# sunshanlu/ORB_SLAM2_ROS2

Hardware: AMD Instinct MI355X
Metric: stereo frames/sec (extract+match) KITTI-00 1241x376; HBM GB/s vs roofline (higher is better)
Workload: dtype u8; 1 GPU; Single 1241x376 KITTI-shaped stereo pair, 8-level pyramid, 2000 FAST+rBRIEF keypoints per image, searchByStereo; batched (512 pairs per step, 512 of them distinct synthetic frames).  `value` is DEVICE-RESIDENT; the checks, rooflines, host_io, sequence job, content sweep, CPU baseline and extra legs run with --full; io=device-resident, n_features=2000, levels=8

## Files before the change

### orb_slam2_ros2_amd/csrc/k_brief.hip

```cpp
#include <hip/hip_runtime.h>
#include <cstdio>
#include <cstring>

#include "orb_math.h"
#include "orbfe_internal.h"
#ifdef BRIEF_STAMPS
namespace orbfe { extern __device__ unsigned long long g_rt_t[4][8]; }
#define RT_STAMP(k) { __syncthreads(); if (tid == 0 && blockIdx.y == 0) orbfe::g_rt_t[k][0] = __builtin_amdgcn_s_memrealtime(); }
#define RTP_STAMP(k) { __syncthreads(); if (tid == 0 && blockIdx.y == 0) orbfe::g_rt_t[k][r] = __builtin_amdgcn_s_memrealtime(); }
#endif
#include "rowtable_body.h"
#include "wave_ops.h"

namespace orbfe {

typedef unsigned long long UmaxPacked;

template <int CTRL, int ROW_MASK>
__device__ __forceinline__ int dpp_i32(int v) {
  return __builtin_amdgcn_update_dpp(0, v, CTRL, ROW_MASK, 0xf, false);
}
__device__ __forceinline__ int wave_sum_i(int v) {
  v += dpp_i32<0x111, 0xf>(v);
  v += dpp_i32<0x112, 0xf>(v);
// ... 247 lines not shown
  orbfe_keypoint kp;
  kp.x = (float)x * L.sf;
  kp.y = (float)y * L.sf;
  kp.size = 7.0f;
  kp.angle = (float)(theta / 3.14159265358979323846 * 180);
  kp.response = (float)((e.y >> 8) & 0xFFu);
  kp.octave = level;
  kp.class_id = -1;
  kps[o] = kp;
#ifndef EXP_NO_KPS_HOST
  if (kps_host) kps_host[o] = kp;
#endif
  kx[o] = kpx_of(kp, L.sf);
  const float r = (float)(2.0 * (double)L.sf);
  const unsigned row = (unsigned)__float2int_rn(kp.y);
  KpAux a;
  a.row_max = (int16_t)min(rows0, __float2int_rn((float)row + r + 1.0f));
  a.row_min = (int16_t)max(0, __float2int_rn((float)row - r));
  aux[o] = a;
  if (theta_out) theta_out[o] = theta;
}

#define BRIEF_R 18
#define BRIEF_ROWS (2 * BRIEF_R + 1)
#define BRIEF_PITCH 48
#define BRIEF_WIN_BYTES 2048

#ifndef BRIEF_WAVES
#define BRIEF_WAVES 4
#endif
#ifndef BRIEF_KPW
#define BRIEF_KPW 2
#endif
#ifdef BRIEF_STAMPS
__device__ unsigned long long g_rt_t[4][8];
__device__ unsigned long long g_bs_rec[8192][6];
#define BS_DECL const unsigned bs_w = ((blockIdx.y * 520u + blockIdx.x) * BRIEF_WAVES + (threadIdx.x >> 6)) & 8191u; const unsigned long long bs_t0 = __builtin_amdgcn_s_memrealtime(); unsigned long long bs_t1 = 0, bs_ta = 0, bs_tb = 0;
#define BS_MID if (!bs_t1) bs_t1 = __builtin_amdgcn_s_memrealtime();
#define BS_END(kind) if ((threadIdx.x & 63) == 0) { asm volatile("s_waitcnt vmcnt(0) lgkmcnt(0)" ::: "memory"); g_bs_rec[bs_w][0] = bs_t0, g_bs_rec[bs_w][1] = bs_t1, g_bs_rec[bs_w][2] = __builtin_amdgcn_s_memrealtime(), g_bs_rec[bs_w][3] = kind, g_bs_rec[bs_w][4] = bs_ta, g_bs_rec[bs_w][5] = bs_tb; }
#else
#define BS_DECL
#define BS_MID
#define BS_END(kind)
#endif
struct BriefRowTable {
  const KpAux* aux;
  const int32_t* n_kp;
  uint32_t* rowoff;
  uint16_t* rowlist;
  int32_t* n_match;
  int rows, list_cap, slot0, n_brief_blocks;
  int stage_cap;
  int32_t* flags;
};
__global__ __launch_bounds__(64 * BRIEF_WAVES) __attribute__((amdgpu_waves_per_eu(8, 8))) void k_brief(const uint8_t* __restrict__ blur, size_t img_pitch,
                                              const uint4* __restrict__ kpl, int n_features, const int8_t* __restrict__ pattern,
                                              const double2* __restrict__ sincos, uint8_t* __restrict__ desc, uint8_t* __restrict__ desc_host,
                                              BriefRowTable rt) {
#pragma clang fp contract(off)
  struct __attribute__((aligned(16))) Lds {
    double rc[BRIEF_WAVES][40];
    uint8_t win[BRIEF_WAVES][2][BRIEF_WIN_BYTES];
    double rs[BRIEF_WAVES][40];
  };
  static_assert(BRIEF_ROWS * BRIEF_PITCH <= BRIEF_WIN_BYTES && BRIEF_WIN_BYTES == 2 * 64 * 16 && BRIEF_PITCH % 16 == 0, "a window is two 16-byte LDS-DMA instructions");
  static_assert((sizeof(double) * 40 * BRIEF_WAVES) % 16 == 0, "the LDS-DMA destination is 16-byte aligned");
  static_assert(sizeof(double) * 40 * BRIEF_WAVES + 2 * BRIEF_WIN_BYTES * BRIEF_WAVES > 255 * 8 &&
                    (sizeof(double) * 40 * BRIEF_WAVES + 2 * BRIEF_WIN_BYTES * BRIEF_WAVES) % 512 != 0,
                "rc[w] and rs[w] must not be reachable by one ds_read2(st64)_b64");
  __shared__ Lds lds;
  BS_DECL
  if (rt.rowoff && (int)blockIdx.x >= rt.n_brief_blocks) {
    static_assert(sizeof(Lds) >= 9000, "the table's row counters borrow the descriptor kernel's LDS (launch_orient_brief checks the row count against 9000 bytes)");
    uint32_t* cnt = (uint32_t*)&lds;
    const int slot = rt.slot0 + (int)blockIdx.y;
    const int r = (int)blockIdx.x - rt.n_brief_blocks;
    if (rt.flags) {
      if (r == 0 && threadIdx.x == 0) rt.n_match[slot >> 1] = 0;
      const int rpw = (rt.rows + 7) >> 3;
      extern __shared__ __attribute__((aligned(16))) uint2 brief_bands[];
      rowtable_build_part(rt.aux + (size_t)blockIdx.y * n_features, min(rt.n_kp[blockIdx.y], n_features), rt.rows, rt.list_cap,
                          rt.rowoff + (size_t)slot * (rt.rows + 1), rt.rowlist + (size_t)slot * rt.list_cap, cnt, cnt + rpw + 12, (int)threadIdx.x, r,
                          rt.flags + (size_t)blockIdx.y * 8, rt.stage_cap > 0 ? brief_bands : nullptr, rt.stage_cap / 4);
      BS_END(2)
      return;
    }
    if (r != 0) return;
    if (threadIdx.x == 0) rt.n_match[slot >> 1] = 0;
    extern __shared__ __attribute__((aligned(16))) uint16_t brief_stage[];
    rowtable_build(rt.aux + (size_t)blockIdx.y * n_features, min(rt.n_kp[blockIdx.y], n_features), rt.rows, rt.list_cap,
                   rt.rowoff + (size_t)slot * (rt.rows + 1), rt.rowlist + (size_t)slot * rt.list_cap, cnt, cnt + rt.rows, (int)threadIdx.x,
                   rt.stage_cap > 0 ? brief_stage : nullptr, rt.stage_cap);
    BS_END(2)
    return;
  }
  const int lane = threadIdx.x & 63;
  const int wave = __builtin_amdgcn_readfirstlane((int)(threadIdx.x >> 6));
  double* rc = lds.rc[wave];
  double* rs = lds.rs[wave];
  const int per_xcd = rt.n_brief_blocks >> 3;
  const int kb = ((int)blockIdx.x & 7) * per_xcd + ((int)blockIdx.x >> 3);
  const int k0 = (kb * BRIEF_WAVES + wave) * BRIEF_KPW;
  const int img = blockIdx.y;
  if (k0 >= n_features) return;
  const uint4* list = kpl + (size_t)img * n_features;
  const double2* sc = sincos + (size_t)img * n_features;
  const uint8_t* W = blur + (size_t)img * img_pitch;
  const int k_last = min(k0 + BRIEF_KPW, n_features) - 1;
  uint32_t tp0 = *(const uint32_t*)(pattern + (0 * 64 + lane) * 4), tp1 = *(const uint32_t*)(pattern + (1 * 64 + lane) * 4);
  uint32_t tp2 = *(const uint32_t*)(pattern + (2 * 64 + lane) * 4), tp3 = *(const uint32_t*)(pattern + (3 * 64 + lane) * 4);
#ifdef BRIEF_STAMPS
  asm volatile("s_waitcnt vmcnt(0)" :: "v"(tp0), "v"(tp1), "v"(tp2), "v"(tp3) : "memory");
  bs_t1 = __builtin_amdgcn_s_memrealtime();
#endif
  const int u1 = min(lane + 64, BRIEF_ROWS * (BRIEF_PITCH / 16) - 1);
  const uint32_t row_a = (uint32_t)lane / 3u, row_b = (uint32_t)u1 / 3u;
  const uint32_t col_a = 16u * ((uint32_t)lane - 3u * row_a), col_b = 16u * ((uint32_t)u1 - 3u * row_b);
  typedef __attribute__((address_space(3))) uint8_t* lds_dst_t;
  typedef const __attribute__((address_space(1))) uint8_t* glb_src_t;
  auto request = [&](const uint4 e, int b) __attribute__((always_inline)) {
    const bool used = (e.x & 0xFFFFu) != 0xFFFFu;
    const int x = used ? (int)(e.x & 0xFFFFu) : BRIEF_R, y = used ? (int)(e.x >> 16) : BRIEF_R;
    const uint32_t plane = used ? e.z : 0u;
    const uint32_t stride = used ? e.w : 0u;
    const uint32_t xa = (uint32_t)(x - BRIEF_R) & ~3u;
    const uint32_t s0 = plane + (uint32_t)(y - BRIEF_R) * stride + xa;
    uint8_t* dst = lds.win[wave][b];
    __builtin_amdgcn_global_load_lds((glb_src_t)(W + (s0 + col_a + __umul24(row_a, stride))), (lds_dst_t)dst, 16, 0, 0);
    __builtin_amdgcn_global_load_lds((glb_src_t)(W + (s0 + col_b + __umul24(row_b, stride))), (lds_dst_t)(dst + 1024), 16, 0, 0);
  };
  uint4 e_cur = list[k0];
  uint4 e_nxt = list[min(k0 + 1, k_last)];
  double2 sc_cur = sc[k0];
#ifdef BRIEF_STAMPS
  asm volatile("s_waitcnt lgkmcnt(0)" ::: "memory");
  bs_ta = __builtin_amdgcn_s_memrealtime();
#endif
  asm volatile("" : "+v"(tp0), "+v"(tp1), "+v"(tp2), "+v"(tp3));
  request(e_cur, 0);
#ifdef BRIEF_STAMPS
  asm volatile("s_waitcnt vmcnt(0)" ::: "memory");
  bs_tb = __builtin_amdgcn_s_memrealtime();
#endif
#pragma unroll
  for (int i = 0; i < BRIEF_KPW; ++i) {
    const int k = k0 + i;
    if (k > k_last) break;
    uint4 e_nn = e_nxt;
    double2 sc_nxt = sc_cur;
    if (i + 2 < BRIEF_KPW) e_nn = list[min(k + 2, k_last)];
    if (i + 1 < BRIEF_KPW && k < k_last) {
      request(e_nxt, (i + 1) & 1);
      sc_nxt = sc[k + 1];
      asm volatile("s_waitcnt vmcnt(2)" ::: "memory");
    } else {
      asm volatile("s_waitcnt vmcnt(0)" ::: "memory");
    }
    __builtin_amdgcn_wave_barrier();
    if ((e_cur.x & 0xFFFFu) != 0xFFFFu) {
      const int x = (int)(e_cur.x & 0xFFFFu), y = (int)(e_cur.x >> 16);
      const int xa = (x - BRIEF_R) & ~3;
      const uint8_t* win = lds.win[wave][i & 1];
      const double sn = sc_cur.x, cs = sc_cur.y;
      if (lane <= 2 * BRIEF_R) {
        const double v = (double)(float)(lane - BRIEF_R);
        rc[lane] = v * cs;
        rs[lane] = v * sn;
      }
      __builtin_amdgcn_fence(__ATOMIC_RELEASE, "wavefront");
      __builtin_amdgcn_wave_barrier();
      BS_MID
      const float px = (float)x, py = (float)y;
      typedef const __attribute__((address_space(3))) uint8_t* lds_bytes_t;
      auto magic_row = [](int y0w) { return (float)(12582912 - (y0w & ~1)); };
      auto magic_col = [](int xa, int y0w, int pitch, int lds_addr) { return (float)(12582912 - xa + lds_addr - (y0w & 1) * pitch); };
      const int y0w = y - BRIEF_R;
      const float magic_y = magic_row(y0w);
      const float magic_x = magic_col(xa, y0w, BRIEF_PITCH, (int)(uint32_t)(uintptr_t)(lds_bytes_t)win);
      auto tests = [&](const uint32_t tpg) __attribute__((always_inline)) -> unsigned long long {
        const int x1 = (int)(int8_t)(tpg & 255u), y1 = (int)(int8_t)((tpg >> 8) & 255u);
        const int x2 = (int)(int8_t)((tpg >> 16) & 255u), y2 = (int)(int8_t)(tpg >> 24);
        const float p1x = (float)(rc[x1 + BRIEF_R] - rs[y1 + BRIEF_R]);
        const float p1y = (float)(rs[x1 + BRIEF_R] + rc[y1 + BRIEF_R]);
        const float p2x = (float)(rc[x2 + BRIEF_R] - rs[y2 + BRIEF_R]);
        const float p2y = (float)(rs[x2 + BRIEF_R] + rc[y2 + BRIEF_R]);
        const uint32_t a1 = (uint32_t)mad24u(__float_as_int((py + p1y) + magic_y), BRIEF_PITCH, __float_as_int((px + p1x) + magic_x)) & 0xFFFFu;
        const uint32_t a2 = (uint32_t)mad24u(__float_as_int((py + p2y) + magic_y), BRIEF_PITCH, __float_as_int((px + p2x) + magic_x)) & 0xFFFFu;
        const int v1 = *(lds_bytes_t)(uintptr_t)a1;
        const int v2 = *(lds_bytes_t)(uintptr_t)a2;
        return __ballot(v1 < v2);
      };
      const unsigned long long bits0 = tests(tp0), bits1 = tests(tp1), bits2 = tests(tp2), bits3 = tests(tp3);
      if (lane < 4) {
        unsigned long long* d64 = (unsigned long long*)(desc + ((size_t)img * n_features + k) * 32);
        unsigned long long b = bits0;
        if (lane == 1) b = bits1;
        if (lane == 2) b = bits2;
        if (lane == 3) b = bits3;
        d64[lane] = b;
        if (desc_host) ((unsigned long long*)(desc_host + ((size_t)img * n_features + k) * 32))[lane] = b;
      }
      __builtin_amdgcn_fence(__ATOMIC_RELEASE, "wavefront");
      __builtin_amdgcn_wave_barrier();
    }
    if (i + 1 < BRIEF_KPW) {
      e_cur = e_nxt;
      e_nxt = e_nn;
      sc_cur = sc_nxt;
    }
  }
  BS_END(1)
}
#ifdef BRIEF_STAMPS
}
extern "C" void orbfe_debug_brief_stamps() {
  static unsigned long long rec[8192][6];
  (void)hipDeviceSynchronize();
  (void)hipMemcpyFromSymbol(rec, HIP_SYMBOL(orbfe::g_bs_rec), sizeof(rec));
  unsigned long long first = ~0ull, last = 0, n = 0, sum = 0, mx = 0, mid = 0, rt0 = 0, rt1 = 0, dlast = 0, sa = 0, sb = 0, ma = 0, mb = 0, smax = 0;
  for (int w = 0; w < 8192; ++w) {
    if (!rec[w][3]) continue;
    first = first < rec[w][0] ? first : rec[w][0], last = last > rec[w][2] ? last : rec[w][2];
    if (rec[w][3] == 1) {
      ++n, sum += rec[w][2] - rec[w][0], mx = mx > rec[w][2] - rec[w][0] ? mx : rec[w][2] - rec[w][0], mid += rec[w][1] ? rec[w][1] - rec[w][0] : 0;
      dlast = dlast > rec[w][2] ? dlast : rec[w][2];
      sa += rec[w][4] - rec[w][0], sb += rec[w][5] - rec[w][4];
      ma = ma > rec[w][4] - rec[w][0] ? ma : rec[w][4] - rec[w][0], mb = mb > rec[w][5] - rec[w][4] ? mb : rec[w][5] - rec[w][4];
    }
  }
  printf("BRIEF stamps (last launch): %llu descriptor waves, launch span %.2f us, last descriptor wave ends at %.2f us; wave mean %.2f max %.2f us, pattern words arrive after %.2f us (mean)\n",
         n, (last - first) * 0.01, (dlast - first) * 0.01, n ? sum * 0.01 / n : 0.0, mx * 0.01, n ? mid * 0.01 / n : 0.0);
  for (int w = 0; w < 8192; ++w)
    if (rec[w][3] == 1) smax = smax > rec[w][0] - first ? smax : rec[w][0] - first;
  printf("  pattern + list entries arrive after %.2f us (mean, max %.2f); window + sin/cos %.2f us later (mean, max %.2f); last descriptor wave starts at %.2f us\n",
         n ? sa * 0.01 / n : 0.0, ma * 0.01, n ? sb * 0.01 / n : 0.0, mb * 0.01, smax * 0.01);
  for (int w = 0; w < 8192; ++w)
    if (rec[w][3] == 2 && (w & 3) == 0) printf("  row-table workgroup: starts %.2f us, ends %.2f us after the launch's first wave\n", (rec[w][0] - first) * 0.01, (rec[w][2] - first) * 0.01);
  {
    unsigned long long rt[4][8];
    (void)hipMemcpyFromSymbol(rt, HIP_SYMBOL(orbfe::g_rt_t), sizeof(rt));
    for (int r = 0; r < 8; ++r)
      printf("  row table part %d (image 0): zeroed %.2f | counted %.2f | lower parts known %.2f | scattered %.2f us after the launch's first wave\n", r,
             (rt[0][r] - first) * 0.01, (rt[1][r] - first) * 0.01, (rt[2][r] - first) * 0.01, (rt[3][r] - first) * 0.01);
  }
  memset(rec, 0, sizeof(rec));
  (void)hipMemcpyToSymbol(HIP_SYMBOL(orbfe::g_bs_rec), rec, sizeof(rec));
  (void)rt0, (void)rt1;
}
namespace orbfe {
#endif

void launch_orient_brief(hipStream_t s, const LevelDev* d_lv, int n_levels, const uint8_t* d_pyr, const uint8_t* d_blur,
                         size_t img_pitch, const uint32_t* d_sel, const int32_t* d_sel_count, int n_features,
                         const int8_t* d_pattern, const int umax[16], orbfe_keypoint* d_kps, uint8_t* d_desc, KpAux* d_aux,
                         int32_t* d_n_kp, double* d_theta, int2* d_moments, double2* d_sincos, KpX* d_kx,
                         uint4* d_kpl, int rows0, int n_img, hipEvent_t before_brief, hipEvent_t before_lists, orbfe_keypoint* h_kps,
                         uint8_t* h_desc, int32_t* h_n_kp, bool fuse_small, uint32_t* d_rowoff_slot, uint16_t* d_rowlist_slot, int32_t* d_n_match,
                         int rt_rows, int rt_list_cap, int rt_slot0, int32_t* d_rt_flags) {
  if (n_img <= 0 || n_features <= 0) return;
  UmaxPacked u = 0;
  for (int i = 0; i < 16; ++i) u |= (unsigned long long)(umax[i] & 15) << (4 * i);
  if (fuse_small && n_img <= 2) {
    if (before_lists) (void)hipStreamWaitEvent(s, before_lists, 0);
    hipLaunchKernelGGL(k_list_moments_orient<true>, dim3((n_features + 15) / 16, n_img), dim3(256), 0, s, d_lv, n_levels, d_sel, d_sel_count, n_features,
                       d_pyr, img_pitch, u, d_kpl, d_moments, d_sincos, d_kps, d_aux, d_kx, d_theta, rows0, d_n_kp, h_kps, h_n_kp,
                       (d_rowoff_slot && d_rt_flags) ? d_rt_flags + (size_t)rt_slot0 * 8 : (int32_t*)nullptr);
    if (before_brief) (void)hipStreamWaitEvent(s, before_brief, 0);
    const int nb = (((n_features + BRIEF_WAVES * BRIEF_KPW - 1) / (BRIEF_WAVES * BRIEF_KPW)) + 7) & ~7;
    BriefRowTable rt{};
    rt.n_brief_blocks = nb;
    if (d_rowoff_slot && (size_t)(rt_rows + 4) * 4 <= 9000)
      rt = BriefRowTable{d_aux, d_n_kp, d_rowoff_slot, d_rowlist_slot, d_n_match, rt_rows, rt_list_cap, rt_slot0, nb, 0,
                         d_rt_flags ? d_rt_flags + (size_t)rt_slot0 * 8 : (int32_t*)nullptr};
    if (rt.rowoff && (rt.flags || rt_list_cap % 8 == 0)) rt.stage_cap = rt.flags ? 4 * std::min(n_features, 4096) : std::min(rt_list_cap, 20480);
    hipLaunchKernelGGL(k_brief, dim3(nb + (rt.rowoff ? 8 : 0), n_img), dim3(64 * BRIEF_WAVES), (size_t)rt.stage_cap * 2, s, d_blur, img_pitch, d_kpl, n_features,
                       d_pattern, d_sincos, d_desc, h_desc, rt);
#ifdef EXP_BRIEF_TWICE
    hipLaunchKernelGGL(k_brief, dim3(nb + (rt.rowoff ? 8 : 0), n_img), dim3(64 * BRIEF_WAVES), 0, s, d_blur, img_pitch, d_kpl, n_features, d_pattern,
                       d_sincos, d_desc, h_desc, rt);
#endif
    return;
  }
  hipLaunchKernelGGL(k_kplist, dim3((n_features + 255) / 256, n_img), dim3(256), 0, s, d_lv, n_levels, d_sel, d_sel_count, n_features,
                     d_kpl);
  hipLaunchKernelGGL(k_ic_moments, dim3((n_features + 15) / 16, n_img), dim3(256), 0, s, d_pyr, img_pitch, d_kpl, n_features, u,
                     d_moments);
  if (before_lists) (void)hipStreamWaitEvent(s, before_lists, 0);
  hipLaunchKernelGGL(k_orient, dim3((n_features + 255) / 256, n_img), dim3(256), 0, s, d_lv, d_kpl, n_features, d_moments, d_sincos,
                     d_kps, d_aux, d_kx, d_theta, rows0, d_sel_count, n_levels, d_n_kp, h_kps, h_n_kp);
  if (before_brief) (void)hipStreamWaitEvent(s, before_brief, 0);
  BriefRowTable rt_none{};
  rt_none.n_brief_blocks = (((n_features + BRIEF_WAVES * BRIEF_KPW - 1) / (BRIEF_WAVES * BRIEF_KPW)) + 7) & ~7;
  hipLaunchKernelGGL(k_brief, dim3(rt_none.n_brief_blocks, n_img), dim3(64 * BRIEF_WAVES), 0, s, d_blur, img_pitch, d_kpl, n_features, d_pattern, d_sincos, d_desc,
                     h_desc, rt_none);
}

}
```

### orb_slam2_ros2_amd/csrc/orbfe_api.hip

```cpp
#include "orbfe_ctx.h"

static const int8_t kEmbeddedPattern[256][4] = {
#include "brief_pattern.inc"
};

static thread_local std::string g_last_error;

orbfe_status fail(orbfe_ctx* c, orbfe_status st, const char* fmt, ...) {
  char buf[512];
  va_list ap;
  va_start(ap, fmt);
  vsnprintf(buf, sizeof buf, fmt, ap);
  va_end(ap);
  (void)c;
  g_last_error = buf;
  return st;
}


static void build_resize_axis(int s, int d, std::vector<ResizeTap>& out) {
  const double scale = 1.0 / ((double)d / s);
  for (int i = 0; i < d; ++i) {
    float f = (float)((i + 0.5) * scale - 0.5);
    int si = cv_floor_f(f);
// ... 580 lines not shown
    fail(c, ORBFE_EDEVICE, "hipSetDevice(%d) failed", c->device);
    return bail(ORBFE_EDEVICE);
  }
  {
    int ncu = 0;
    if (hipDeviceGetAttribute(&ncu, hipDeviceAttributeMultiprocessorCount, c->device) == hipSuccess && ncu > 0) c->n_cu = ncu;
  }
  if (cfg->stream) {
    c->stream = (hipStream_t)cfg->stream;
  } else {
    if (hipStreamCreateWithFlags(&c->stream, hipStreamNonBlocking) != hipSuccess) {
      fail(c, ORBFE_EDEVICE, "hipStreamCreate failed");
      return bail(ORBFE_EDEVICE);
    }
    c->own_stream = true;
  }
  c->main.stream = c->stream;
  c->slot_lane.resize((size_t)cfg->max_images);
  {
    if (const char* gr = getenv("ORBFE_GRAPHS")) c->use_graphs = atoi(gr) != 0;
    {
      const char* ps = getenv("ORBFE_PIPELINE_STEREO");
      c->pipeline_stereo = !ps || atoi(ps) != 0;
      if (c->pipeline_stereo &&
          (hipStreamCreateWithFlags(&c->stereo_stream, hipStreamNonBlocking) != hipSuccess ||
           hipEventCreateWithFlags(&c->ev_brief_done, hipEventDisableTiming) != hipSuccess ||
           hipEventCreateWithFlags(&c->ev_stereo_done, hipEventDisableTiming) != hipSuccess)) {
        fail(c, ORBFE_EDEVICE, "cannot create the stereo stream");
        return bail(ORBFE_EDEVICE);
      }
    }
    if (const char* hl = getenv("ORBFE_LBA_HOST_LM")) c->lm_on_device = atoi(hl) == 0;
    if (const char* fc = getenv("ORBFE_FAST_CPW")) c->fast_cpw = std::max(0, std::min(64, atoi(fc)));
    if (const char* fm = getenv("ORBFE_FAST_SIDE_MASK")) c->fast_side_mask = (int64_t)(strtoul(fm, nullptr, 0) & 0xFFFFu);
    if (const char* fg = getenv("ORBFE_FAST_SIDE_MERGE")) c->fast_side_merge = atoi(fg) != 0;
    const char* ov = getenv("ORBFE_OVERLAP_BLUR");
    if (!ov || atoi(ov) != 0) {
      if (hipStreamCreateWithFlags(&c->blur_stream, hipStreamNonBlocking) != hipSuccess ||
          hipEventCreateWithFlags(&c->ev_blur_go, hipEventDisableTiming) != hipSuccess ||
          hipEventCreateWithFlags(&c->ev_blur_done, hipEventDisableTiming) != hipSuccess) {
        fail(c, ORBFE_EDEVICE, "cannot create the blur stream");
        return bail(ORBFE_EDEVICE);
      }
      if (c->fast_side_mask != 0 && cfg->max_images >= 32 &&
          (hipStreamCreateWithFlags(&c->fast_stream, hipStreamNonBlocking) != hipSuccess ||
           hipEventCreateWithFlags(&c->ev_fast_go, hipEventDisableTiming) != hipSuccess ||
           hipEventCreateWithFlags(&c->ev_fast_side_done, hipEventDisableTiming) != hipSuccess)) {
        fail(c, ORBFE_EDEVICE, "cannot create the FAST side stream");
        return bail(ORBFE_EDEVICE);
      }
    }
  }
  const size_t M = (size_t)cfg->max_images, NF = (size_t)std::max(c->cfg.n_features, 1), NL = (size_t)cfg->n_levels;
  const size_t NP = (M + 1) / 2;
#define ALLOC(ptr, count)                          \
  do {                                             \
    st = dev_alloc(c, &(ptr), (count));            \
    if (st != ORBFE_OK) return bail(st);           \
  } while (0)
  ALLOC(c->d_lv, NL);
  ALLOC(c->d_cells, c->cells.size());
  ALLOC(c->d_taps, c->taps.size());
  ALLOC(c->d_rs_tiles, c->rs_tile_tab.size());
  ALLOC(c->d_rs_regions, std::max<size_t>(c->rs_regions.size(), 1));
  ALLOC(c->d_rg_xtaps, std::max<size_t>(c->rg_xtaps.size(), 2));
  ALLOC(c->d_rg_ytaps, std::max<size_t>(c->rg_ytaps.size(), 1));
// ... 318 lines not shown
```

### orb_slam2_ros2_amd/csrc/orbfe_ctx.h

```cpp
#pragma once
#include <hip/hip_runtime.h>
#include <sched.h>

#include <algorithm>
#include <cctype>
#include <cmath>
#include <cstdarg>
#include <cstdio>
#include <cstdlib>
#include <cstring>
#include <atomic>
#include <chrono>
#include <mutex>
#include <string>
#include <limits>
#include <memory>
#include <vector>

#include "orbfe_internal.h"
#include "scratch_layout.h"
#include "staged_rows.h"
#include "search_area_layout.h"

namespace orbfe {
void launch_resize(hipStream_t s, const LevelDev* d_lv, const RsTile* d_tiles, const int* n_tiles, const int* lds_bytes,
                   const ResizeTap* d_taps, uint8_t* d_pyr,
                   size_t img_pitch, int n_img);
void launch_resize_regions(hipStream_t s, const LevelDev* d_lv, int n_levels, const RsRegion* d_regions, int n_regions, int tile_bytes,
                           int xt_bytes, int yt_bytes, const RgXTap* d_xtaps, const RgYTap* d_ytaps, uint8_t* d_pyr, size_t img_pitch, int n_img,
                           const uint8_t* src_a, const uint8_t* src_b, size_t src_pitch, int src_stride, uint32_t src_bytes, int copy_l0, int32_t* d_zero, int n_zero, int pq, int32_t* d_zero2 = nullptr, int n_zero2 = 0);
void launch_blur(hipStream_t s, const LevelDev* d_lv, int n_levels, int tile_first, int n_tiles, const uint8_t* d_pyr, uint8_t* d_blur,
                 size_t img_pitch, const int taps[7], int n_img);
bool mb_build(const LevelDev* lv, int n_levels, const int taps[7], uint32_t spare_off, MbGeom* g, std::vector<uint8_t>* tx, std::vector<uint8_t>* ty);
void launch_blur_mfma(hipStream_t s, const LevelDev* d_lv, int n_levels, const MbGeom& g, const uint8_t* d_pyr, uint8_t* d_blur, size_t img_pitch,
                      const uint8_t* d_tx, const uint8_t* d_ty, int n_img);
void launch_load_level0(hipStream_t st, const uint8_t* d_src, const uint8_t* d_src_b, size_t src_stride, size_t src_pitch, uint8_t* d_pyr,
                        size_t img_pitch, uint32_t plane_off, int dst_stride, int w, int h, int slot0, int slot_step, int n_img);
void launch_fast(hipStream_t s, const LevelDev* d_lv, const CellDev* d_cells, const LevelDev* h_lv, const int* lvl_max_pw,
                 const int* lvl_max_ph, const uint8_t* d_pyr, size_t img_pitch, int t_hi, int t_lo, uint32_t* d_cand, size_t cand_pitch,
                 int32_t* d_n_cand, int n_levels, int n_img, int cpw_force, uint32_t level_mask = ~0u, bool merge_masked = false,
                 int32_t* d_n_cand_sh = nullptr, int n_shards = 1);
bool fast_single_launch(const LevelDev* h_lv, const int* lvl_max_pw, const int* lvl_max_ph, int n_levels, int n_img);
size_t quadtree_lds_bytes(int node_cap, int rec_cap, int sort_cap);
hipError_t quadtree_configure(size_t lds_bytes);
void launch_quadtree(hipStream_t s, const LevelDev* d_lv, int n_levels, const uint32_t* d_cand, uint32_t* d_scr_b, uint32_t* d_scr_c,
                     size_t scratch_pitch, uint32_t* d_sel, int32_t* d_sel_count, int n_features, const int32_t* d_n_cand, int node_cap, int sort_cap,
                     int rec_cap, int n_img, int batch, const QtGroups& groups, int n_groups, int waves_per_tree, uint8_t* d_big, size_t big_pitch,
                     const uint16_t* d_qt_tabs, const uint8_t* blur_pyr, uint8_t* blur_out, size_t img_pitch, const int* blur_taps, int blur_tiles,
                     int32_t* d_qt_next, bool next_zeroed = false, const int32_t* d_n_cand_sh = nullptr, int n_shards = 1);
bool quadtree_build_tables(const LevelDev& L, std::vector<uint16_t>& out);
void launch_orient_brief(hipStream_t s, const LevelDev* d_lv, int n_levels, const uint8_t* d_pyr, const uint8_t* d_blur,
                         size_t img_pitch, const uint32_t* d_sel, const int32_t* d_sel_count, int n_features,
                         const int8_t* d_pattern, const int umax[16], orbfe_keypoint* d_kps, uint8_t* d_desc, KpAux* d_aux,
                         int32_t* d_n_kp, double* d_theta, int2* d_moments, double2* d_sincos, KpX* d_kx,
                         uint4* d_kpl, int rows0, int n_img, hipEvent_t before_brief, hipEvent_t before_lists, orbfe_keypoint* h_kps, uint8_t* h_desc, int32_t* h_n_kp,
                         bool fuse_small, uint32_t* d_rowoff_slot = nullptr, uint16_t* d_rowlist_slot = nullptr,
                         int32_t* d_n_match = nullptr, int rt_rows = 0, int rt_list_cap = 0, int rt_slot0 = 0, int32_t* d_rt_flags = nullptr);
void launch_match_bruteforce(hipStream_t s, const uint8_t* d_q, int nq, const uint8_t* d_t, int nt, const uint32_t* d_off,
                             const uint32_t* d_cand, int32_t* d_best_idx, int32_t* d_best_dist, int32_t* d_second);
void launch_stereo(hipStream_t s, const LevelDev* d_lv, int n_levels, const uint8_t* d_pyr, size_t img_pitch, const orbfe_keypoint* d_kps,
                   const uint8_t* d_desc, const KpAux* d_aux, const KpX* d_kx, uint32_t* d_rowoff, uint16_t* d_rowlist, int rows, int list_cap,
                   const int32_t* d_n_kp, int n_features, float fx, float bf, int cols0, int mean_threshold, double* d_right_u, double* d_depth, int32_t* d_n_match, int32_t* d_best_right,
                   int32_t* d_best_dist, int slot_l0, int slot_r0, int slot_step, int pair0, int n_pairs, double* h_right_u, double* h_depth,
                   int32_t* h_best_right, int32_t* h_best_dist, bool table_ready = false, const StereoRowsBuf* rowsbuf = nullptr);
void launch_cvt_gray(hipStream_t s, const uint8_t* d_src, size_t src_stride, uint8_t* d_dst, int dst_stride, int w, int h, int order,
                     int variant);
void launch_frame_rgbd(hipStream_t s, orbfe_keypoint* d_kps, const int32_t* d_n_kp, int n_features, const orbfe_camera& cam,
                       const uint8_t* d_depth, int depth_type, size_t depth_stride, float depth_scale, double* d_depth_out, double* d_right_u, orbfe_keypoint* h_kps = nullptr);
void launch_pack_records(hipStream_t s, const uint8_t* d_kps, const uint8_t* d_desc, const int32_t* d_counts, const uint8_t* d_ru,
                         const uint8_t* d_dp, const int32_t* d_nm, int nf, int n_pairs, void* d_out);
void launch_lba_chi2_sum(hipStream_t s, int n_edges, const double* chi2, const double* rho, const uint8_t* level, double* chi2_last,
                         double* out);
void launch_lba_maxdiag(hipStream_t s, int n_poses, int n_points, const double* Hpp, const double* Hll, const uint8_t* fixed, double* out);
void launch_lba_solve(hipStream_t s, int n_poses, int n_points, int n_edges, int nf, const int32_t* free_pose, const int32_t* pose_slot,
                      const int32_t* pair_off, const int2* pairs, const int32_t* ps_off, const int32_t* ps_edges, const int32_t* pt_off,
                      const int32_t* pt_edges, const int32_t* edge_pose, const int32_t* edge_point, const uint8_t* fixed, const double* Hpp,
                      const double* bp, const double* Hll, const double* bl, const double* Hpl, const double* lambda_p, double* Dinv, double* W,
                      double* S, double* rhs, double* x, int* ok, double* poses, double* points, double* dxp, double* dxl, double* scale_out,
                      double* big_scratch);
void launch_lba_chol(hipStream_t s, int nf, double* S, double* rhs, double* x, int* ok, double* big_scratch);
void launch_lba_pre(hipStream_t s, int n_points, int n_edges, const int32_t* edge_point, const double* Hll, const double* Hpl,
                    const double* lambda_p, double* Dinv, double* W, int* ok);
void launch_lba_post(hipStream_t s, int n_poses, int n_points, const int32_t* pose_slot, const int32_t* pt_off, const int32_t* pt_edges,
                     const int32_t* edge_pose, const uint8_t* fixed, const double* bp, const double* bl, const double* Hpl, const double* lambda_p,
                     const double* Dinv, const double* x, double* poses, double* points, double* dxp, double* dxl, double* scale_out);
void launch_bsr_schur(hipStream_t s, int n_low, const int32_t* low, const int32_t* low_row, const int32_t* col, const int32_t* twin,
                      const int32_t* pair_off, const int2* pairs, const int32_t* free_pose, const int32_t* ps_off, const int32_t* ps_edges,
                      const int32_t* edge_point, const double* Hpp, const double* bp, const double* bl, const double* Hpl, const double* W,
                      const double* lambda_p, double* blocks, double* rhs, double* Minv, int* ok);
void launch_bsr_diag_inv(hipStream_t s, const BsrPcgLaunch& L);
// ... 87 lines not shown
    hipStream_t stream = nullptr;
    bool own_stream = false;
    hipEvent_t ev_main = nullptr;
    uint8_t* h_stage = nullptr;
    size_t h_stage_bytes = 0;
    std::vector<GraphEntry> graphs;
    bool use_graphs = true;
    std::atomic<bool> pending{false};
  };
  struct HostStream {
    static const int kDepth = 3;
    bool init = false;
    hipStream_t h2d = nullptr, d2h = nullptr;
    uint8_t* d_in[kDepth] = {nullptr, nullptr, nullptr};
    size_t in_bytes = 0;
    uint8_t* d_out[kDepth] = {nullptr, nullptr, nullptr};
    size_t out_bytes = 0;
    hipEvent_t ev_h2d[kDepth] = {nullptr, nullptr, nullptr}, ev_in_free[kDepth] = {nullptr, nullptr, nullptr},
               ev_out_ready[kDepth] = {nullptr, nullptr, nullptr}, ev_done[kDepth] = {nullptr, nullptr, nullptr};
    int64_t next_ticket = 0;
    int32_t n_pairs_of[kDepth] = {0, 0, 0};
  } hs;
  Lane main;
  std::vector<std::unique_ptr<Lane>> slot_lane;
  std::mutex slot_lane_mu;
  bool use_graphs = true;
  uint8_t* d_pyr_alt = nullptr;
  hipStream_t stereo_stream = nullptr;
  hipEvent_t ev_brief_done = nullptr, ev_stereo_done = nullptr;
  std::atomic<bool> stereo_pending{false};
  bool pipeline_stereo = true;
  hipStream_t blur_stream = nullptr;
  int fast_cpw = 0;
  hipEvent_t ev_blur_go = nullptr, ev_blur_done = nullptr;
  int64_t fast_side_mask = -1;
  bool fast_side_merge = false;
  hipStream_t fast_stream = nullptr;
  hipEvent_t ev_fast_go = nullptr, ev_fast_side_done = nullptr;

  std::vector<LevelDev> lv;
  std::vector<CellDev> cells;
  std::vector<ResizeTap> taps;
  std::vector<RsTile> rs_tile_tab;
  RsTile* d_rs_tiles = nullptr;
  int umax[16];
  int blur_taps[7];
  int n_cells_total = 0, rs_tiles = 0, bl_tiles = 0;
  int kp_cap = 0;
  std::vector<RsRegion> rs_regions;
  RsRegion* d_rs_regions = nullptr;
  std::vector<RgXTap> rg_xtaps;
  std::vector<RgYTap> rg_ytaps;
  RgXTap* d_rg_xtaps = nullptr;
  RgYTap* d_rg_ytaps = nullptr;
  int rg_tile_bytes = 0, rg_xt_bytes = 0, rg_yt_bytes = 0;
  int rg_pq = 0;
  int rs_n[3] = {0, 0, 0}, rs_bytes[3] = {0, 0, 0};
  size_t img_pitch = 0;
  size_t scratch_pitch = 0;
  QtGroups qt_groups_of[3];
  uint32_t pyr_spare_off = 0;
  MbGeom mb = {};
  bool mb_ok = false;
  uint8_t *d_mb_tx = nullptr, *d_mb_ty = nullptr;
  std::vector<uint8_t> mb_tx, mb_ty;
  int32_t* d_qt_next = nullptr;
// ... 239 lines not shown
```

### orb_slam2_ros2_amd/csrc/orbfe_extract.hip

```cpp
#include "orbfe_ctx.h"
void grid_invalidate(orbfe_ctx* c, int slot) {
  if (!c->grid_key) return;
  std::atomic<uint64_t>& a = c->grid_key[(size_t)slot];
  uint64_t v = a.load();
  while (!a.compare_exchange_weak(v, ((v >> 32) + 1) << 32)) {
  }
}
static bool fast_lists_sharded(const orbfe_ctx* c, int n_img) {
  const int nl = c->cfg.n_levels;
  return c->fast_shards > 1 && c->d_n_cand_sh && fast_single_launch(c->lv.data(), c->lvl_max_pw, c->lvl_max_ph, nl, n_img) &&
         (long long)nl * n_img <= c->n_cu;
}
void note_slots_written(orbfe_ctx* c, int s0, int n, bool small) {
  for (int s = s0; s < s0 + n && s < c->cfg.max_images; ++s) grid_invalidate(c, s);
  const bool sharded = fast_lists_sharded(c, n);
  for (int s = s0; s < s0 + n && s < c->cfg.max_images; ++s) c->slot_sharded[(size_t)s] = sharded ? 1 : 0;
  if (!c->slot_table_ok) return;
  for (int s = s0; s < s0 + n && s < c->cfg.max_images; ++s) {
    c->slot_table_ok[(size_t)s] = small ? 1 : 0;
    if (small) c->pair_count_zero[(size_t)(s >> 1)] = 1;
  }
}
orbfe_status run_extract(orbfe_ctx* c, hipStream_t st, int img0, int n_img, hipEvent_t before_lists, bool timing, const ExtLevel0* ext,
                         const HostMirror* mirror) {
// ... 96 lines not shown
    StageTimer t(c, ORBFE_STAGE_QUADTREE, st, timing);
    int gsel = -1;
    if (nl > 4) {
      const long long per8 = (long long)c->n_cu * 16;
      if ((long long)n_img * 1 >= per8) gsel = 0;
      else if ((long long)n_img * 2 >= per8) gsel = 1;
      else if ((long long)n_img * 4 >= per8) gsel = 2;
    }
    const bool grouped = gsel >= 0;
    const int n_groups = gsel >= 0 ? std::min(nl, 1 << gsel) : nl;
    const QtGroups& qt_tab = gsel >= 0 ? c->qt_groups_of[gsel] : c->qt_single;
    const int trees = n_groups * n_img;
    const int per_cu = (trees + c->n_cu - 1) / c->n_cu;
    const size_t lds_cu = 160 * 1024 - 2048;
    const size_t node_bytes = quadtree_lds_bytes(c->node_cap, 0, c->sort_cap);
    size_t budget = lds_cu / (size_t)std::max(per_cu, 1);
    budget -= budget % 512;
    const int rec_cap = budget > node_bytes ? (int)std::min<size_t>((budget - node_bytes) / 4, (size_t)c->rec_cap) : 0;
    launch_quadtree(st, c->d_lv, nl, c->d_scr_a + i0 * c->scratch_pitch, c->d_scr_b + i0 * c->scratch_pitch,
                    c->d_scr_c + i0 * c->scratch_pitch, c->scratch_pitch, c->d_sel + i0 * NF, c->d_sel_count + i0 * nl,
                    c->cfg.n_features, n_cand, c->node_cap, c->sort_cap, rec_cap, n_img, 1, qt_tab, n_groups,
                    (!grouped && trees * 4 <= c->n_cu * 4) ? 4 : 1, c->d_qt_big ? c->d_qt_big + i0 * c->qt_big_pitch : nullptr,
                    c->qt_big_pitch, c->d_qt_tabs, blur_in_qt ? pyr : nullptr, blur, c->img_pitch, c->blur_taps, c->bl_tiles, c->d_qt_next + i0,
                    zeroed_by_resize && !sharded, n_cand_sh, sharded ? c->fast_shards : 1);
  }
  {
    StageTimer t(c, ORBFE_STAGE_BRIEF, st, timing);
    launch_orient_brief(st, c->d_lv, nl, pyr, blur, c->img_pitch, c->d_sel + i0 * NF, c->d_sel_count + i0 * nl, c->cfg.n_features,
                        c->d_pattern, c->umax, c->d_kps + i0 * NF, c->d_desc + i0 * NF * 32, c->d_aux + i0 * NF, c->d_n_kp + i0,
                        c->d_theta + i0 * NF, c->d_moments + i0 * NF, c->d_sincos + i0 * NF, c->d_kx + i0 * NF,
                        c->d_kpl + i0 * NF, c->cfg.height, n_img,
                        overlap_blur ? c->ev_blur_done : nullptr, before_lists, mirror ? mirror->kps : nullptr, mirror ? mirror->desc : nullptr,
                        mirror ? mirror->n_kp : nullptr, true, n_img <= 2 ? c->d_rowoff_slot : nullptr, c->d_rowlist_slot, c->d_n_match, c->cfg.height,
                        c->row_list_cap, img0, n_img <= 2 ? c->d_rt_flags : nullptr);
  }
  HIP_TRY(c, hipGetLastError());
  return ORBFE_OK;
}

struct StereoHostOut {
  double *right_u, *depth;
  int32_t *best_right, *best_dist;
};
static orbfe_status run_stereo(orbfe_ctx* c, hipStream_t st, int slot_l0, int slot_r0, int slot_step, int pair0, int n_pairs, float fx,
                               float bf, const StereoHostOut* ho = nullptr, bool table_ready = false, bool timing = true) {
  {
    StageTimer t(c, ORBFE_STAGE_STEREO, st, timing);
    launch_stereo(st, c->d_lv, c->cfg.n_levels, c->d_pyr, c->img_pitch, c->d_kps, c->d_desc, c->d_aux, c->d_kx,
                  table_ready ? c->d_rowoff_slot : c->d_rowoff, table_ready ? c->d_rowlist_slot : c->d_rowlist,
                  c->cfg.height, c->row_list_cap, c->d_n_kp,
                  c->cfg.n_features, fx, bf,
                  c->cfg.width, kMeanThreshold, c->d_right_u, c->d_depth, c->d_n_match, c->d_best_right, c->d_best_dist, slot_l0,
                  slot_r0, slot_step, pair0, n_pairs, ho ? ho->right_u : nullptr, ho ? ho->depth : nullptr, ho ? ho->best_right : nullptr,
                  ho ? ho->best_dist : nullptr, table_ready, &c->st_rows);
  }
  HIP_TRY(c, hipGetLastError());
  return ORBFE_OK;
}

extern "C" {


static orbfe_status enqueue_fetch(orbfe_ctx* c, orbfe_ctx::Lane& ln, int slot0, int n_img, size_t o_kps, size_t o_desc, size_t o_cnt,
                                  bool want_kps, bool want_desc) {
  const size_t NF = (size_t)std::max(c->cfg.n_features, 1), s0 = (size_t)slot0;
  HIP_TRY(c, hipMemcpyAsync(ln.h_stage + o_cnt, c->d_n_kp + s0, sizeof(int32_t) * n_img, hipMemcpyDeviceToHost, ln.stream));
  if (want_kps)
// ... 478 lines not shown
```

Baseline: 119,200 stereo pairs/s.

## Make BRIEF keypoints-per-wave a runtime loop with strided assignment and precomputed LDS addresses

Replaces the compile-time unrolled BRIEF_KPW loop with a runtime, non-unrolled loop in which each wave handles keypoints strided by the wave count. The batched path now defaults to 3 keypoints per wave, and the count can be overridden through an environment variable. The pattern's LDS table addresses are precomputed once into registers, the address math is done in inline asm (mad24 with pitch 48 plus a mask), and the descriptor is written by 8 lanes via v_writelane instead of 4 lanes with 64-bit stores. The XCD block swizzle also now mixes in blockIdx.y. The aim is to amortise per-wave setup over more keypoints and cut VALU work per test, at the cost of fewer blocks and higher register pressure.

```diff
diff --git a/orb_slam2_ros2_amd/csrc/k_brief.hip b/orb_slam2_ros2_amd/csrc/k_brief.hip
--- a/orb_slam2_ros2_amd/csrc/k_brief.hip
+++ b/orb_slam2_ros2_amd/csrc/k_brief.hip
@@ -303,6 +303,16 @@
 #ifndef BRIEF_KPW
 #define BRIEF_KPW 2
 #endif
+#ifndef BRIEF_KPW_BATCH
+#define BRIEF_KPW_BATCH 3
+#endif
+#define BRIEF_KPW_MAX 64
+__device__ __forceinline__ uint32_t brief_addr(int row_bits, int col_bits) {
+  static_assert(BRIEF_PITCH == 48, "the pitch is spelled out in the instruction");
+  uint32_t d;
+  asm("v_mad_u32_u24 %0, %1, 48, %2\n\tv_and_b32 %0, 0xffff, %0" : "=v"(d) : "v"(row_bits), "v"(col_bits));
+  return d;
+}
 #ifdef BRIEF_STAMPS
 __device__ unsigned long long g_rt_t[4][8];
 __device__ unsigned long long g_bs_rec[8192][6];
@@ -327,7 +337,7 @@
 __global__ __launch_bounds__(64 * BRIEF_WAVES) __attribute__((amdgpu_waves_per_eu(8, 8))) void k_brief(const uint8_t* __restrict__ blur, size_t img_pitch,
                                               const uint4* __restrict__ kpl, int n_features, const int8_t* __restrict__ pattern,
                                               const double2* __restrict__ sincos, uint8_t* __restrict__ desc, uint8_t* __restrict__ desc_host,
-                                              BriefRowTable rt) {
+                                              BriefRowTable rt, int kpw) {
 #pragma clang fp contract(off)
   struct __attribute__((aligned(16))) Lds {
     double rc[BRIEF_WAVES][40];
@@ -367,62 +377,74 @@
   }
   const int lane = threadIdx.x & 63;
   const int wave = __builtin_amdgcn_readfirstlane((int)(threadIdx.x >> 6));
-  double* rc = lds.rc[wave];
-  double* rs = lds.rs[wave];
   const int per_xcd = rt.n_brief_blocks >> 3;
-  const int kb = ((int)blockIdx.x & 7) * per_xcd + ((int)blockIdx.x >> 3);
-  const int k0 = (kb * BRIEF_WAVES + wave) * BRIEF_KPW;
+  const int kb = (((int)blockIdx.x + (int)blockIdx.y) & 7) * per_xcd + ((int)blockIdx.x >> 3);
+  const int kbase = kb * (BRIEF_WAVES * kpw) + wave;
   const int img = blockIdx.y;
-  if (k0 >= n_features) return;
+  if (kbase >= n_features) return;
+  const int k_last = kbase + BRIEF_WAVES * (min(kpw, (n_features - kbase + BRIEF_WAVES - 1) / BRIEF_WAVES) - 1);
   const uint4* list = kpl + (size_t)img * n_features;
   const double2* sc = sincos + (size_t)img * n_features;
   const uint8_t* W = blur + (size_t)img * img_pitch;
-  const int k_last = min(k0 + BRIEF_KPW, n_features) - 1;
-  uint32_t tp0 = *(const uint32_t*)(pattern + (0 * 64 + lane) * 4), tp1 = *(const uint32_t*)(pattern + (1 * 64 + lane) * 4);
-  uint32_t tp2 = *(const uint32_t*)(pattern + (2 * 64 + lane) * 4), tp3 = *(const uint32_t*)(pattern + (3 * 64 + lane) * 4);
-#ifdef BRIEF_STAMPS
-  asm volatile("s_waitcnt vmcnt(0)" :: "v"(tp0), "v"(tp1), "v"(tp2), "v"(tp3) : "memory");
-  bs_t1 = __builtin_amdgcn_s_memrealtime();
-#endif
-  const int u1 = min(lane + 64, BRIEF_ROWS * (BRIEF_PITCH / 16) - 1);
-  const uint32_t row_a = (uint32_t)lane / 3u, row_b = (uint32_t)u1 / 3u;
-  const uint32_t col_a = 16u * ((uint32_t)lane - 3u * row_a), col_b = 16u * ((uint32_t)u1 - 3u * row_b);
   typedef __attribute__((address_space(3))) uint8_t* lds_dst_t;
   typedef const __attribute__((address_space(1))) uint8_t* glb_src_t;
-  auto request = [&](const uint4 e, int b) __attribute__((always_inline)) {
+  typedef const __attribute__((address_space(3))) uint8_t* lds_bytes_t;
+  typedef const __attribute__((address_space(3))) double* lds_f64_t;
+  typedef __attribute__((address_space(3))) double* lds_f64w_t;
+  const uint32_t rc_addr = (uint32_t)(uintptr_t)(lds_bytes_t)(const uint8_t*)lds.rc[wave];
+  const uint32_t win_addr = (uint32_t)(uintptr_t)(lds_bytes_t)lds.win[wave][0];
+  constexpr uint32_t RS_OFF = (uint32_t)(sizeof(double) * 40 * BRIEF_WAVES + 2 * BRIEF_WIN_BYTES * BRIEF_WAVES);
+  static_assert(RS_OFF < 65536, "the distance of the two tables is a ds_read offset");
+  uint32_t ta0, ta1, ta2, ta3, ta4, ta5, ta6, ta7, ta8, ta9, ta10, ta11, ta12, ta13, ta14, ta15;
+  {
+    const uint32_t tp0 = *(const uint32_t*)(pattern + (0 * 64 + lane) * 4), tp1 = *(const uint32_t*)(pattern + (1 * 64 + lane) * 4);
+    const uint32_t tp2 = *(const uint32_t*)(pattern + (2 * 64 + lane) * 4), tp3 = *(const uint32_t*)(pattern + (3 * 64 + lane) * 4);
+    auto entry = [&](uint32_t tpg, int byte) { return rc_addr + (uint32_t)(((int)(int8_t)((tpg >> (8 * byte)) & 255u) + BRIEF_R) * 8); };
+    ta0 = entry(tp0, 0), ta1 = entry(tp0, 1), ta2 = entry(tp0, 2), ta3 = entry(tp0, 3);
+    ta4 = entry(tp1, 0), ta5 = entry(tp1, 1), ta6 = entry(tp1, 2), ta7 = entry(tp1, 3);
+    ta8 = entry(tp2, 0), ta9 = entry(tp2, 1), ta10 = entry(tp2, 2), ta11 = entry(tp2, 3);
+    ta12 = entry(tp3, 0), ta13 = entry(tp3, 1), ta14 = entry(tp3, 2), ta15 = entry(tp3, 3);
+  }
+  const int u1 = min(lane + 64, BRIEF_ROWS * (BRIEF_PITCH / 16) - 1);
+  uint32_t row_a = (uint32_t)lane / 3u, row_b = (uint32_t)u1 / 3u;
+  uint32_t col_a = 16u * ((uint32_t)lane - 3u * row_a), col_b = 16u * ((uint32_t)u1 - 3u * row_b);
+  double tv = (double)(float)(lane - BRIEF_R);
+  uint32_t tw_addr = rc_addr + 8u * (uint32_t)lane;
+  uint32_t st_off = 4u * (uint32_t)lane;
+  auto request = [&](const uint4 e, uint32_t wo) __attribute__((always_inline)) {
     const bool used = (e.x & 0xFFFFu) != 0xFFFFu;
     const int x = used ? (int)(e.x & 0xFFFFu) : BRIEF_R, y = used ? (int)(e.x >> 16) : BRIEF_R;
     const uint32_t plane = used ? e.z : 0u;
     const uint32_t stride = used ? e.w : 0u;
     const uint32_t xa = (uint32_t)(x - BRIEF_R) & ~3u;
     const uint32_t s0 = plane + (uint32_t)(y - BRIEF_R) * stride + xa;
-    uint8_t* dst = lds.win[wave][b];
-    __builtin_amdgcn_global_load_lds((glb_src_t)(W + (s0 + col_a + __umul24(row_a, stride))), (lds_dst_t)dst, 16, 0, 0);
-    __builtin_amdgcn_global_load_lds((glb_src_t)(W + (s0 + col_b + __umul24(row_b, stride))), (lds_dst_t)(dst + 1024), 16, 0, 0);
+    lds_dst_t dst = (lds_dst_t)(uintptr_t)(win_addr + wo);
+    __builtin_amdgcn_global_load_lds((glb_src_t)(W + (s0 + col_a + __umul24(row_a, stride))), dst, 16, 0, 0);
+    __builtin_amdgcn_global_load_lds((glb_src_t)(W + (s0 + col_b + __umul24(row_b, stride))), dst + 1024, 16, 0, 0);
   };
-  uint4 e_cur = list[k0];
-  uint4 e_nxt = list[min(k0 + 1, k_last)];
-  double2 sc_cur = sc[k0];
+  int k = kbase;
+  uint4 e_cur = list[k];
+  uint4 e_nxt = list[min(k + BRIEF_WAVES, k_last)];
+  double2 sc_cur = sc[k];
 #ifdef BRIEF_STAMPS
   asm volatile("s_waitcnt lgkmcnt(0)" ::: "memory");
   bs_ta = __builtin_amdgcn_s_memrealtime();
 #endif
-  asm volatile("" : "+v"(tp0), "+v"(tp1), "+v"(tp2), "+v"(tp3));
-  request(e_cur, 0);
+  asm volatile("" : "+v"(ta0), "+v"(ta1), "+v"(ta2), "+v"(ta3), "+v"(ta4), "+v"(ta5), "+v"(ta6), "+v"(ta7), "+v"(ta8), "+v"(ta9), "+v"(ta10),
+               "+v"(ta11), "+v"(ta12), "+v"(ta13), "+v"(ta14), "+v"(ta15), "+v"(row_a), "+v"(row_b), "+v"(col_a), "+v"(col_b), "+v"(tv),
+               "+v"(tw_addr), "+v"(st_off));
+  request(e_cur, 0u);
 #ifdef BRIEF_STAMPS
   asm volatile("s_waitcnt vmcnt(0)" ::: "memory");
   bs_tb = __builtin_amdgcn_s_memrealtime();
 #endif
-#pragma unroll
-  for (int i = 0; i < BRIEF_KPW; ++i) {
-    const int k = k0 + i;
-    if (k > k_last) break;
-    uint4 e_nn = e_nxt;
-    double2 sc_nxt = sc_cur;
-    if (i + 2 < BRIEF_KPW) e_nn = list[min(k + 2, k_last)];
-    if (i + 1 < BRIEF_KPW && k < k_last) {
-      request(e_nxt, (i + 1) & 1);
-      sc_nxt = sc[k + 1];
+  uint32_t wo = 0u;
+#pragma clang loop unroll(disable)
+  for (;;) {
+    const uint4 e_nn = list[min(k + 2 * BRIEF_WAVES, k_last)];
+    const double2 sc_nxt = sc[min(k + BRIEF_WAVES, k_last)];
+    if (k < k_last) {
+      request(e_nxt, wo ^ BRIEF_WIN_BYTES);
       asm volatile("s_waitcnt vmcnt(2)" ::: "memory");
     } else {
       asm volatile("s_waitcnt vmcnt(0)" ::: "memory");
@@ -431,54 +453,57 @@
     if ((e_cur.x & 0xFFFFu) != 0xFFFFu) {
       const int x = (int)(e_cur.x & 0xFFFFu), y = (int)(e_cur.x >> 16);
       const int xa = (x - BRIEF_R) & ~3;
-      const uint8_t* win = lds.win[wave][i & 1];
       const double sn = sc_cur.x, cs = sc_cur.y;
       if (lane <= 2 * BRIEF_R) {
-        const double v = (double)(float)(lane - BRIEF_R);
-        rc[lane] = v * cs;
-        rs[lane] = v * sn;
+        *(lds_f64w_t)(uintptr_t)tw_addr = tv * cs;
+        *(lds_f64w_t)(uintptr_t)(tw_addr + RS_OFF) = tv * sn;
       }
       __builtin_amdgcn_fence(__ATOMIC_RELEASE, "wavefront");
       __builtin_amdgcn_wave_barrier();
       BS_MID
       const float px = (float)x, py = (float)y;
-      typedef const __attribute__((address_space(3))) uint8_t* lds_bytes_t;
       auto magic_row = [](int y0w) { return (float)(12582912 - (y0w & ~1)); };
       auto magic_col = [](int xa, int y0w, int pitch, int lds_addr) { return (float)(12582912 - xa + lds_addr - (y0w & 1) * pitch); };
       const int y0w = y - BRIEF_R;
       const float magic_y = magic_row(y0w);
-      const float magic_x = magic_col(xa, y0w, BRIEF_PITCH, (int)(uint32_t)(uintptr_t)(lds_bytes_t)win);
-      auto tests = [&](const uint32_t tpg) __attribute__((always_inline)) -> unsigned long long {
-        const int x1 = (int)(int8_t)(tpg & 255u), y1 = (int)(int8_t)((tpg >> 8) & 255u);
-        const int x2 = (int)(int8_t)((tpg >> 16) & 255u), y2 = (int)(int8_t)(tpg >> 24);
-        const float p1x = (float)(rc[x1 + BRIEF_R] - rs[y1 + BRIEF_R]);
-        const float p1y = (float)(rs[x1 + BRIEF_R] + rc[y1 + BRIEF_R]);
-        const float p2x = (float)(rc[x2 + BRIEF_R] - rs[y2 + BRIEF_R]);
-        const float p2y = (float)(rs[x2 + BRIEF_R] + rc[y2 + BRIEF_R]);
-        const uint32_t a1 = (uint32_t)mad24u(__float_as_int((py + p1y) + magic_y), BRIEF_PITCH, __float_as_int((px + p1x) + magic_x)) & 0xFFFFu;
-        const uint32_t a2 = (uint32_t)mad24u(__float_as_int((py + p2y) + magic_y), BRIEF_PITCH, __float_as_int((px + p2x) + magic_x)) & 0xFFFFu;
+      const float magic_x = magic_col(xa, y0w, BRIEF_PITCH, (int)(win_addr + wo));
+      auto tests = [&](uint32_t ax1, uint32_t ay1, uint32_t ax2, uint32_t ay2) __attribute__((always_inline)) -> unsigned long long {
+        const double c_x1 = *(lds_f64_t)(uintptr_t)ax1, s_y1 = *(lds_f64_t)(uintptr_t)(ay1 + RS_OFF);
+        const double s_x1 = *(lds_f64_t)(uintptr_t)(ax1 + RS_OFF), c_y1 = *(lds_f64_t)(uintptr_t)ay1;
+        const double c_x2 = *(lds_f64_t)(uintptr_t)ax2, s_y2 = *(lds_f64_t)(uintptr_t)(ay2 + RS_OFF);
+        const double s_x2 = *(lds_f64_t)(uintptr_t)(ax2 + RS_OFF), c_y2 = *(lds_f64_t)(uintptr_t)ay2;
+        const float p1x = (float)(c_x1 - s_y1);
+        const float p1y = (float)(s_x1 + c_y1);
+        const float p2x = (float)(c_x2 - s_y2);
+        const float p2y = (float)(s_x2 + c_y2);
+        const uint32_t a1 = brief_addr(__float_as_int((py + p1y) + magic_y), __float_as_int((px + p1x) + magic_x));
+        const uint32_t a2 = brief_addr(__float_as_int((py + p2y) + magic_y), __float_as_int((px + p2x) + magic_x));
         const int v1 = *(lds_bytes_t)(uintptr_t)a1;
         const int v2 = *(lds_bytes_t)(uintptr_t)a2;
         return __ballot(v1 < v2);
       };
-      const unsigned long long bits0 = tests(tp0), bits1 = tests(tp1), bits2 = tests(tp2), bits3 = tests(tp3);
-      if (lane < 4) {
-        unsigned long long* d64 = (unsigned long long*)(desc + ((size_t)img * n_features + k) * 32);
-        unsigned long long b = bits0;
-        if (lane == 1) b = bits1;
-        if (lane == 2) b = bits2;
-        if (lane == 3) b = bits3;
-        d64[lane] = b;
-        if (desc_host) ((unsigned long long*)(desc_host + ((size_t)img * n_features + k) * 32))[lane] = b;
+      const unsigned long long bits0 = tests(ta0, ta1, ta2, ta3), bits1 = tests(ta4, ta5, ta6, ta7);
+      const unsigned long long bits2 = tests(ta8, ta9, ta10, ta11), bits3 = tests(ta12, ta13, ta14, ta15);
+      uint32_t dv;
+      asm("v_writelane_b32 %0, %1, 0\n\tv_writelane_b32 %0, %2, 1\n\tv_writelane_b32 %0, %3, 2\n\tv_writelane_b32 %0, %4, 3\n\t"
+          "v_writelane_b32 %0, %5, 4\n\tv_writelane_b32 %0, %6, 5\n\tv_writelane_b32 %0, %7, 6\n\tv_writelane_b32 %0, %8, 7"
+          : "=v"(dv)
+          : "s"((uint32_t)bits0), "s"((uint32_t)(bits0 >> 32)), "s"((uint32_t)bits1), "s"((uint32_t)(bits1 >> 32)), "s"((uint32_t)bits2),
+            "s"((uint32_t)(bits2 >> 32)), "s"((uint32_t)bits3), "s"((uint32_t)(bits3 >> 32)));
+      if (lane < 8) {
+        const size_t o = ((size_t)img * n_features + k) * 32;
+        *(uint32_t*)(desc + o + st_off) = dv;
+        if (desc_host) *(uint32_t*)(desc_host + o + st_off) = dv;
       }
       __builtin_amdgcn_fence(__ATOMIC_RELEASE, "wavefront");
       __builtin_amdgcn_wave_barrier();
     }
-    if (i + 1 < BRIEF_KPW) {
-      e_cur = e_nxt;
-      e_nxt = e_nn;
-      sc_cur = sc_nxt;
-    }
+    if (k >= k_last) break;
+    k += BRIEF_WAVES;
+    wo ^= BRIEF_WIN_BYTES;
+    e_cur = e_nxt;
+    e_nxt = e_nn;
+    sc_cur = sc_nxt;
   }
   BS_END(1)
 }
@@ -527,7 +552,7 @@
                          int32_t* d_n_kp, double* d_theta, int2* d_moments, double2* d_sincos, KpX* d_kx,
                          uint4* d_kpl, int rows0, int n_img, hipEvent_t before_brief, hipEvent_t before_lists, orbfe_keypoint* h_kps,
                          uint8_t* h_desc, int32_t* h_n_kp, bool fuse_small, uint32_t* d_rowoff_slot, uint16_t* d_rowlist_slot, int32_t* d_n_match,
-                         int rt_rows, int rt_list_cap, int rt_slot0, int32_t* d_rt_flags) {
+                         int rt_rows, int rt_list_cap, int rt_slot0, int32_t* d_rt_flags, int brief_kpw) {
   if (n_img <= 0 || n_features <= 0) return;
   UmaxPacked u = 0;
   for (int i = 0; i < 16; ++i) u |= (unsigned long long)(umax[i] & 15) << (4 * i);
@@ -537,7 +562,8 @@
                        d_pyr, img_pitch, u, d_kpl, d_moments, d_sincos, d_kps, d_aux, d_kx, d_theta, rows0, d_n_kp, h_kps, h_n_kp,
                        (d_rowoff_slot && d_rt_flags) ? d_rt_flags + (size_t)rt_slot0 * 8 : (int32_t*)nullptr);
     if (before_brief) (void)hipStreamWaitEvent(s, before_brief, 0);
-    const int nb = (((n_features + BRIEF_WAVES * BRIEF_KPW - 1) / (BRIEF_WAVES * BRIEF_KPW)) + 7) & ~7;
+    const int kpw = brief_kpw > 0 ? std::min(brief_kpw, BRIEF_KPW_MAX) : BRIEF_KPW;
+    const int nb = (((n_features + BRIEF_WAVES * kpw - 1) / (BRIEF_WAVES * kpw)) + 7) & ~7;
     BriefRowTable rt{};
     rt.n_brief_blocks = nb;
     if (d_rowoff_slot && (size_t)(rt_rows + 4) * 4 <= 9000)
@@ -545,10 +571,10 @@
                          d_rt_flags ? d_rt_flags + (size_t)rt_slot0 * 8 : (int32_t*)nullptr};
     if (rt.rowoff && (rt.flags || rt_list_cap % 8 == 0)) rt.stage_cap = rt.flags ? 4 * std::min(n_features, 4096) : std::min(rt_list_cap, 20480);
     hipLaunchKernelGGL(k_brief, dim3(nb + (rt.rowoff ? 8 : 0), n_img), dim3(64 * BRIEF_WAVES), (size_t)rt.stage_cap * 2, s, d_blur, img_pitch, d_kpl, n_features,
-                       d_pattern, d_sincos, d_desc, h_desc, rt);
+                       d_pattern, d_sincos, d_desc, h_desc, rt, kpw);
 #ifdef EXP_BRIEF_TWICE
     hipLaunchKernelGGL(k_brief, dim3(nb + (rt.rowoff ? 8 : 0), n_img), dim3(64 * BRIEF_WAVES), 0, s, d_blur, img_pitch, d_kpl, n_features, d_pattern,
-                       d_sincos, d_desc, h_desc, rt);
+                       d_sincos, d_desc, h_desc, rt, kpw);
 #endif
     return;
   }
@@ -561,9 +587,10 @@
                      d_kps, d_aux, d_kx, d_theta, rows0, d_sel_count, n_levels, d_n_kp, h_kps, h_n_kp);
   if (before_brief) (void)hipStreamWaitEvent(s, before_brief, 0);
   BriefRowTable rt_none{};
-  rt_none.n_brief_blocks = (((n_features + BRIEF_WAVES * BRIEF_KPW - 1) / (BRIEF_WAVES * BRIEF_KPW)) + 7) & ~7;
+  const int kpw = brief_kpw > 0 ? std::min(brief_kpw, BRIEF_KPW_MAX) : BRIEF_KPW_BATCH;
+  rt_none.n_brief_blocks = (((n_features + BRIEF_WAVES * kpw - 1) / (BRIEF_WAVES * kpw)) + 7) & ~7;
   hipLaunchKernelGGL(k_brief, dim3(rt_none.n_brief_blocks, n_img), dim3(64 * BRIEF_WAVES), 0, s, d_blur, img_pitch, d_kpl, n_features, d_pattern, d_sincos, d_desc,
-                     h_desc, rt_none);
-}
-
-}
+                     h_desc, rt_none, kpw);
+}
+
+}
diff --git a/orb_slam2_ros2_amd/csrc/orbfe_api.hip b/orb_slam2_ros2_amd/csrc/orbfe_api.hip
--- a/orb_slam2_ros2_amd/csrc/orbfe_api.hip
+++ b/orb_slam2_ros2_amd/csrc/orbfe_api.hip
@@ -636,6 +636,7 @@
     }
     if (const char* hl = getenv("ORBFE_LBA_HOST_LM")) c->lm_on_device = atoi(hl) == 0;
     if (const char* fc = getenv("ORBFE_FAST_CPW")) c->fast_cpw = std::max(0, std::min(64, atoi(fc)));
+    if (const char* bk = getenv("ORBFE_BRIEF_KPW")) c->brief_kpw = std::max(0, std::min(64, atoi(bk)));
     if (const char* fm = getenv("ORBFE_FAST_SIDE_MASK")) c->fast_side_mask = (int64_t)(strtoul(fm, nullptr, 0) & 0xFFFFu);
     if (const char* fg = getenv("ORBFE_FAST_SIDE_MERGE")) c->fast_side_merge = atoi(fg) != 0;
     const char* ov = getenv("ORBFE_OVERLAP_BLUR");
diff --git a/orb_slam2_ros2_amd/csrc/orbfe_ctx.h b/orb_slam2_ros2_amd/csrc/orbfe_ctx.h
--- a/orb_slam2_ros2_amd/csrc/orbfe_ctx.h
+++ b/orb_slam2_ros2_amd/csrc/orbfe_ctx.h
@@ -55,7 +55,8 @@
                          int32_t* d_n_kp, double* d_theta, int2* d_moments, double2* d_sincos, KpX* d_kx,
                          uint4* d_kpl, int rows0, int n_img, hipEvent_t before_brief, hipEvent_t before_lists, orbfe_keypoint* h_kps, uint8_t* h_desc, int32_t* h_n_kp,
                          bool fuse_small, uint32_t* d_rowoff_slot = nullptr, uint16_t* d_rowlist_slot = nullptr,
-                         int32_t* d_n_match = nullptr, int rt_rows = 0, int rt_list_cap = 0, int rt_slot0 = 0, int32_t* d_rt_flags = nullptr);
+                         int32_t* d_n_match = nullptr, int rt_rows = 0, int rt_list_cap = 0, int rt_slot0 = 0, int32_t* d_rt_flags = nullptr,
+                         int brief_kpw = 0);
 void launch_match_bruteforce(hipStream_t s, const uint8_t* d_q, int nq, const uint8_t* d_t, int nt, const uint32_t* d_off,
                              const uint32_t* d_cand, int32_t* d_best_idx, int32_t* d_best_dist, int32_t* d_second);
 void launch_stereo(hipStream_t s, const LevelDev* d_lv, int n_levels, const uint8_t* d_pyr, size_t img_pitch, const orbfe_keypoint* d_kps,
@@ -209,6 +210,7 @@
   bool pipeline_stereo = true;
   hipStream_t blur_stream = nullptr;
   int fast_cpw = 0;
+  int brief_kpw = 0;
   hipEvent_t ev_blur_go = nullptr, ev_blur_done = nullptr;
   int64_t fast_side_mask = -1;
   bool fast_side_merge = false;
diff --git a/orb_slam2_ros2_amd/csrc/orbfe_extract.hip b/orb_slam2_ros2_amd/csrc/orbfe_extract.hip
--- a/orb_slam2_ros2_amd/csrc/orbfe_extract.hip
+++ b/orb_slam2_ros2_amd/csrc/orbfe_extract.hip
@@ -152,7 +152,7 @@
                         c->d_kpl + i0 * NF, c->cfg.height, n_img,
                         overlap_blur ? c->ev_blur_done : nullptr, before_lists, mirror ? mirror->kps : nullptr, mirror ? mirror->desc : nullptr,
                         mirror ? mirror->n_kp : nullptr, true, n_img <= 2 ? c->d_rowoff_slot : nullptr, c->d_rowlist_slot, c->d_n_match, c->cfg.height,
-                        c->row_list_cap, img0, n_img <= 2 ? c->d_rt_flags : nullptr);
+                        c->row_list_cap, img0, n_img <= 2 ? c->d_rt_flags : nullptr, c->brief_kpw);
   }
   HIP_TRY(c, hipGetLastError());
   return ORBFE_OK;
```

New measurement: 120,500 stereo pairs/s, median of 6. 1.2% higher.
